# ziotom78/pytracer

Hardware: AMD Instinct MI355X
Metric: Mray/s (primary+shadow; rays handed to a world query) at 1280x720 per GPU, C2: 32 spheres + 1 plane, FlatRenderer (higher is better)
Workload: dtype f64; 1 GPU; C2 flat 1280x720, 32 spheres + 1 plane, S=0, every primary ray traced (dome shortcut off), fp32 RGB resident in HBM; width=1280, height=720, renderer=FlatRenderer

## Files before the change

pytracer_amd/csrc/pt_kernels.h:

```cpp
#pragma once
#include <hip/hip_runtime.h>
#include <stdint.h>

#include "../../include/ptrace.h"
#include "pt_layout.h"

#define PT_DEV static __device__ __forceinline__
#define PT_PI 3.141592653589793
#define PT_BLOCK 256
#ifndef PT_WAVES_SIMPLE
#define PT_WAVES_SIMPLE 4
#endif
#ifndef PT_WAVES_TILE
#define PT_WAVES_TILE 4
#endif
#ifndef PT_REGION
#define PT_REGION 8
#endif

typedef const __attribute__((address_space(4))) double *pt_kdouble;
typedef const __attribute__((address_space(4))) int32_t *pt_kint;
#define PT_KD(p) ((pt_kdouble)(const void *)(p))
#define PT_KI(p) ((pt_kint)(const void *)(p))

typedef const __attribute__((address_space(4))) PtKArgs *pt_kargs;
PT_DEV pt_kargs cold_args(const PtKArgs &a) {
  unsigned long long p = (unsigned long long)a.cold;
  asm volatile("" : "+s"(p));
  return (pt_kargs)p;
}

#ifndef PT_QUEUE_WORDS
#define PT_QUEUE_WORDS 512
#endif
#define PT_QUEUE_HEADS 256
#define PT_Q_CHOICE 200
#define PT_Q_HEAVY 201
#define PT_Q_BUDGET 202
#define PT_HANDOVER_HEADER 8
#ifndef PT_UNIT_SHARDS
#define PT_UNIT_SHARDS 8
#endif
static_assert(PT_QUEUE_HEADS + 32 * PT_UNIT_SHARDS <= PT_QUEUE_WORDS, "the shard heads must lie inside the queue block");
PT_DEV unsigned long long *pt_queue(const PtKArgs &a) { return cold_args(a)->queue + (size_t)a.qpar * PT_QUEUE_WORDS; }
PT_DEV unsigned long long *pt_queue_next(const PtKArgs &a) { return cold_args(a)->queue + (size_t)(a.qpar ^ 1) * PT_QUEUE_WORDS; }

struct V3 {
  double x, y, z;
};
struct Ray {
  V3 o, d;
  double tmin;
};
struct Hit {
  V3 wp, n;
  double u, v;
};

#include "pt_math.h"
#include "pt_query.h"
#include "pt_shade.h"
#include "pt_camera.h"
#include "pt_simple.h"
#include "pt_tile.h"
#include "pt_hits.h"
#include "pt_path.h"
#include "pt_tree.h"
#include "pt_probes.h"
```

pytracer_amd/csrc/pt_shade.h:

```cpp
template <bool INL = false, typename RP = const PtShapeRec *, typename AP = const PtShapeAux *>
PT_DEV void hit_details(RP rec, AP ax, const Ray &r, double t, Hit &h, bool need_uv) {
  double im[12];
#pragma unroll
  for (int k = 0; k < 12; ++k) im[k] = rec->invm[k];
  const V3 o = xf_point(im, r.o);
  const V3 d = xf_vec(im, r.d);
  const V3 hp = {o.x + t * d.x, o.y + t * d.y, o.z + t * d.z};
  double fm[12];
#pragma unroll
  for (int k = 0; k < 12; ++k) fm[k] = ax->m[k];
  h.wp = xf_point(fm, hp);
  V3 nn;
  h.u = 0.0;
  h.v = 0.0;
  if (rec->kind == PT_SHAPE_SPHERE) {
    const bool keep = dot3(hp, d) < 0.0;
    nn.x = keep ? hp.x : -hp.x;
    nn.y = keep ? hp.y : -hp.y;
    nn.z = keep ? hp.z : -hp.z;
    if (need_uv) {
      const double uu = pt_atan2(hp.y, hp.x) / (2.0 * PT_PI);
      h.u = (uu >= 0.0) ? uu : uu + 1.0;
      double z = hp.z;
      z = (z > 1.0) ? 1.0 : ((z < -1.0) ? -1.0 : z);
      h.v = pt_acos(z) / PT_PI;
    }
  } else {
    nn.x = 0.0;
    nn.y = 0.0;
    nn.z = (d.z < 0.0) ? 1.0 : -1.0;
    if (need_uv) {
      h.u = hp.x - floor(hp.x);
      h.v = hp.y - floor(hp.y);
    }
  }
  h.n = normalize3(xf_normal(im, nn));
}

template <typename CP>
PT_DEV V3 pigment_color(const PtKArgs &a, int kind, CP c1, CP c2, double steps, int tex, double u, double v) {
  if (kind == PT_PIGMENT_IMAGE) {
    pt_kargs ca = cold_args(a);
    const PtTex *tx = ca->tex + tex;
    const int w = tx->w, hh = tx->h;
    long long col = (long long)(u * (double)w);
    long long row = (long long)(v * (double)hh);
    if (col >= w) col = w - 1;
    if (row >= hh) row = hh - 1;
    const double *c = ca->tex_data + tx->offset + (row * w + col) * 3;
    V3 r = {c[0], c[1], c[2]};
    return r;
  }
  CP c = c1;
  if (kind == PT_PIGMENT_CHECKERED) {
    const double tu = floor(u * steps), tv = floor(v * steps);
    const bool odd_u = floor(tu * 0.5) * 2.0 != tu, odd_v = floor(tv * 0.5) * 2.0 != tv;
    c = (odd_u == odd_v) ? c1 : c2;
  }
  V3 r = {c[0], c[1], c[2]};
  return r;
}
template <typename AP>
PT_DEV V3 brdf_pigment(const PtKArgs &a, AP ax, double u, double v) {
  return pigment_color(a, ax->pig_kind, &ax->pig_c1[0], &ax->pig_c2[0], ax->pig_steps, ax->pig_tex, u, v);
}
template <typename AP>
PT_DEV V3 emitted_pigment(const PtKArgs &a, AP ax, double u, double v) {
  return pigment_color(a, ax->emi_kind, &ax->emi_c1[0], &ax->emi_c2[0], ax->emi_steps, ax->emi_tex, u, v);
}

template <bool INL = false>
PT_DEV Ray scatter_ray(int brdf_kind, Pcg &pcg, V3 incoming, V3 point, V3 n) {
  Ray r;
  r.o = point;
  if (brdf_kind == PT_BRDF_DIFFUSE) {
    const double sign = (n.z > 0.0) ? 1.0 : -1.0;
    const double aa = -1.0 / (sign + n.z);
    const double bb = n.x * n.y * aa;
    const V3 e1 = {1.0 + sign * n.x * n.x * aa, sign * bb, -sign * n.x};
    const V3 e2 = {bb, sign + n.y * n.y * aa, -n.y};
    const double cts = pcg_float(pcg);
    const double ct = sqrt(cts), st = sqrt(1.0 - cts);
    const double phi = 2.0 * PT_PI * pcg_float(pcg);
    double cp, sp;
    if (INL)
      sincos(phi, &sp, &cp);
    else
      pt_sincos(phi, &sp, &cp);
    r.d.x = ct * (cp * e1.x) + ct * (sp * e2.x) + st * n.x;
    r.d.y = ct * (cp * e1.y) + ct * (sp * e2.y) + st * n.y;
    r.d.z = ct * (cp * e1.z) + ct * (sp * e2.z) + st * n.z;
    r.tmin = 1.0e-3;
  } else {
    const V3 rd = normalize3(incoming);
    const V3 nn = normalize3(n);
    const double dp = dot3(nn, rd);
    r.d.x = rd.x - dp * (2.0 * nn.x);
    r.d.y = rd.y - dp * (2.0 * nn.y);
    r.d.z = rd.z - dp * (2.0 * nn.z);
    r.tmin = 1e-5;
  }
  return r;
}

PT_NOINLINE void scatter_ray_call(int brdf_kind, Pcg *pcg, const V3 *incoming, const V3 *point, const V3 *n, Ray *out) {
  *out = scatter_ray(brdf_kind, *pcg, *incoming, *point, *n);
}
```

pytracer_amd/csrc/pt_tile.h:

```cpp
struct TileCone {
  float ox, oy, oz;
  float ax, ay, az;
  float cos_t, sin_t;
  float oabs;
  bool all;
  float kx, ky, kz;
  float dmax2;
  float dmin;
  float rbeam;
  bool ortho;
};

struct ConeCam {
  float d0[3], dx[3], dy[3], apex[3];
  bool ortho;
};

PT_DEV ConeCam cone_cam(const PtKArgs &a) {
  ConeCam k;
  pt_kargs c = cold_args(a);
  for (int i = 0; i < 3; ++i) {
    k.d0[i] = c->cone_d0[i];
    k.dx[i] = c->cone_dx[i];
    k.dy[i] = c->cone_dy[i];
// ... 475 lines not shown
   bool strip_dome = block_dome, strip_settled = block_settled;
   if (use_strips && !block_dome) strip_dome = shared_cull(tx_first, tx_end, ty * 8, ty * 8 + 7, strip_cum, strip_settled);
   {
    const int tx = tx_first + wib;
    if (tx >= tx_end) continue;
    const int tile = ty * tiles_x + tx;
    PT_TSTAMP(7);
    const int col = tx * 8 + (lane & 7), lrow = ty * 8 + (lane >> 3);
    const bool active = col < W && lrow < rows_local;
    const int ccol = col < W ? col : W - 1, clrow = lrow < rows_local ? lrow : rows_local - 1;
    const long long pix = (long long)clrow * W + ccol;
    if (strip_dome) {
      if (strip_settled && active) {
        store_pixel(a, pix, KEEP ? dc_cum : strip_cum, out_f32);
        nrays += (unsigned long long)nsamp;
        nres += (unsigned long long)nsamp;
      }
      if (RENDERER == PT_RENDERER_PATHTRACER) {
        const unsigned long long todo = strip_settled ? 0ULL : __ballot(active);
        if (lane == 0) {
          rmask[tile] = todo;
          rkeys[tile] = (unsigned char)__popcll(todo);
            if (todo) note_flagged(pt_queue(a), __popcll(todo));
        }
      }
      continue;
    }
    const int pcol = ccol, grow = global_row(a, clrow);

    PT_TSTAMP(0);
    const int gr0 = global_row(a, ty * 8);
    const int gr1 = global_row(a, (ty * 8 + 7 < rows_local) ? ty * 8 + 7 : rows_local - 1);
    const float4 b_first = KEEP ? b_kept : a.bounds[(!HIER && lane < a.n_shapes) ? lane : 0];
    const TileCone tc = tile_cone(a, tx * 8, (tx * 8 + 8 < W) ? tx * 8 + 8 : W, gr0, gr1);
    PT_TSTAMP(1);
    int tpass = npass;
    const unsigned int *list = nullptr;
    int list_cnt = 0;
    int nsurv = 0, only = 0;
    bool dome_here = false;
    if (HIER) {
      const int cell = __builtin_amdgcn_readfirstlane((gr0 / PT_CELL) * a.cells_x + (tx * 8) / PT_CELL);
      const int cnt = PT_KI(a.cell_count)[cell];
      list_cnt = cnt;
      list = a.cell_list + (size_t)cell * a.cell_stride;
      tpass = (cnt + 63) >> 6;
      for (int p = 0; p < tpass; ++p) {
        const int idx = p * 64 + lane;
        bool keep = false;
        int slot = 0;
        float4 b = {0.0f, 0.0f, 0.0f, -1.0f};
        if (idx < cnt) {
          slot = (int)list[idx];
          b = a.bounds[slot];
        }
        const bool isplane = idx < cnt && slot >= a.n_spheres;
        if (idx < cnt && !isplane) keep = cone_keeps(tc, b);
        if (__any(isplane)) {
          const bool pk = plane_keeps(tc, b, isplane);
          if (isplane) keep = pk;
        }
        const unsigned long long m = __ballot(keep);
        if (lane == 0) pt_lds_masks[mbase + p] = m;
        nsurv += __popcll(m);
        if (m) only = (int)list[p * 64 + (__ffsll((long long)m) - 1)];
        if (RENDERER == PT_RENDERER_PATHTRACER && __ballot(keep && slot == dome_slot)) dome_here = true;
      }
    } else {
      for (int p = 0; p < npass; ++p) {
        const int slot = p * 64 + lane;
        bool keep = false;
        float4 b = {0.0f, 0.0f, 0.0f, -1.0f};
        if (slot < a.n_shapes) b = p == 0 ? b_first : a.bounds[slot];
        const bool isplane = slot >= a.n_spheres && slot < a.n_shapes;
        if (slot < a.n_spheres) keep = cone_keeps(tc, b);
        if (__any(isplane)) {
          const bool pk = plane_keeps(tc, b, isplane);
          if (isplane) keep = pk;
        }
        const unsigned long long m = __ballot(keep);
        if (lane == 0) pt_lds_masks[mbase + p] = m;
        nsurv += __popcll(m);
        if (m) only = p * 64 + (__ffsll((long long)m) - 1);
        if (RENDERER == PT_RENDERER_PATHTRACER && p == (dome_slot >> 6) && ((m >> (dome_slot & 63)) & 1ULL)) dome_here = true;
      }
    }
    __builtin_amdgcn_fence(__ATOMIC_RELEASE, "wavefront");
    __builtin_amdgcn_wave_barrier();
    __builtin_amdgcn_fence(__ATOMIC_ACQUIRE, "wavefront");
    PT_TSTAMP(2);

    if (dome_on && nsurv == 1 && only < a.n_spheres) {
      only = __builtin_amdgcn_readfirstlane(only);
      double hc_;
      float dmax2 = tc.dmax2, dmin = tc.dmin;
      if (ORTHO) {
        const float fro2 = (float)PT_KD(&a.recs[only])[13];
        pt_kdouble m = PT_KD(a.recs[only].invm);
        const float ox = (float)m[0] * tc.kx + (float)m[1] * tc.ky + (float)m[2] * tc.kz + (float)m[3];
        const float oy = (float)m[4] * tc.kx + (float)m[5] * tc.ky + (float)m[6] * tc.kz + (float)m[7];
        const float oz = (float)m[8] * tc.kx + (float)m[9] * tc.ky + (float)m[10] * tc.kz + (float)m[11];
        float o2 = ox * ox + oy * oy + oz * oz;
        o2 = fmaxf(o2, __shfl_xor(o2, 1, 64));
        o2 = fmaxf(o2, __shfl_xor(o2, 2, 64));
        const float slack = 1e-5f * (fro2 * (tc.oabs * tc.oabs * 3.0f + 1.0f) + 1.0f);
        hc_ = (o2 + slack < 0.45f) ? -0.55 : 0.0;
        pt_kargs cc_ = cold_args(a);
        const float d2 = cc_->cone_apex[0] * cc_->cone_apex[0] + cc_->cone_apex[1] * cc_->cone_apex[1] +
                         cc_->cone_apex[2] * cc_->cone_apex[2];
        dmax2 = d2 * (1.0f + 1e-5f);
        dmin = __fsqrt_rn(d2) * (1.0f - 1e-5f);
      } else {
        hc_ = 0.0;
      }
      V3 cum;
      bool settled;
      if (dome_value(only, hc_, dmax2, dmin, tc.all, cum, settled)) {
        if (settled && active) {
          store_pixel(a, pix, cum, out_f32);
          nrays += (unsigned long long)nsamp;
          nres += (unsigned long long)nsamp;
        }
        if (RENDERER == PT_RENDERER_PATHTRACER) {
          const unsigned long long todo = settled ? 0ULL : __ballot(active);
          if (lane == 0) {
            rmask[tile] = todo;
            rkeys[tile] = (unsigned char)__popcll(todo);
            if (todo) note_flagged(pt_queue(a), __popcll(todo));
          }
        }
        __builtin_amdgcn_wave_barrier();
        continue;
      }
    }

    if (RENDERER == PT_RENDERER_PATHTRACER && !ORTHO && dome_on && dome_here && nsurv > 1) {
      dome_prepare(dome_slot);
      if (dc_usable && dc_settled && dc_hc < -0.5 && dc_fro2 * tc.dmax2 < 1e6f && tc.dmin > 1e-6f && !tc.all) {
        const TileCone pc = pixel_cone(cone_cam(a), tc, pcol, grow);
        bool hitable = pc.all;
        for (int p = 0; p < tpass; ++p) {
          const unsigned long long mv = pt_lds_masks[mbase + p];
          const unsigned m_hi = (unsigned)__builtin_amdgcn_readfirstlane((int)(unsigned)(mv >> 32));
          const unsigned m_lo = (unsigned)__builtin_amdgcn_readfirstlane((int)(unsigned)mv);
          unsigned long long mask = ((unsigned long long)m_hi << 32) | (unsigned long long)m_lo;
          if (!mask) continue;
          const int myi = p * 64 + lane;
          int slot_q = myi;
          if (HIER) slot_q = myi < list_cnt ? (int)list[myi] : 0;
          const float4 bq = a.bounds[slot_q < a.n_shapes ? slot_q : 0];
          while (mask) {
            const int bit = __ffsll((long long)mask) - 1;
            mask &= mask - 1;
            const int slot = __builtin_amdgcn_readlane(slot_q, bit);
            if (slot == dome_slot) continue;
            if (slot >= a.n_spheres) {
              hitable = true;
            } else {
              const float4 b = {__int_as_float(__builtin_amdgcn_readlane(__float_as_int(bq.x), bit)),
                                __int_as_float(__builtin_amdgcn_readlane(__float_as_int(bq.y), bit)),
                                __int_as_float(__builtin_amdgcn_readlane(__float_as_int(bq.z), bit)),
                                __int_as_float(__builtin_amdgcn_readlane(__float_as_int(bq.w), bit))};
              hitable = hitable || cone_keeps(pc, b);
            }
          }
        }
        const V3 cum = dc_cum;
        if (active && !hitable) {
          store_pixel(a, pix, cum, out_f32);
          nrays += (unsigned long long)nsamp;
          nres += (unsigned long long)nsamp;
        }
        const unsigned long long todo = __ballot(active && hitable);
        if (lane == 0) {
          rmask[tile] = todo;
          rkeys[tile] = (unsigned char)__popcll(todo);
            if (todo) note_flagged(pt_queue(a), __popcll(todo));
        }
        __builtin_amdgcn_wave_barrier();
        continue;
      }
    }

    Pcg pcg;
    unsigned long long gpix = 0;
    if (S > 0) {
      pt_kargs c = cold_args(a);
      gpix = (unsigned long long)grow * c->W + pcol;
      pcg_seed_pixel(pcg, c->pcg_mode, c->s0, c->q0, gpix, nsamp);
    }
    V3 cum = {0.0, 0.0, 0.0};
    bool alive = active;
    int pix_rays = 0;
    for (int s = 0; s < nsamp; ++s) {
      if (RENDERER == PT_RENDERER_PATHTRACER && !__any(alive)) break;
      double up = 0.5, vp = 0.5;
      if (S > 0) {
        pt_kargs c = cold_args(a);
        if (c->pcg_mode == PT_PCG_SAMPLE) pcg_seed(pcg, c->s0, c->q0 + gpix * (unsigned)nsamp + (unsigned)s);
        const int sr = s / S, sc = s - sr * S;
        up = ((double)sc + pcg_float(pcg)) / (double)S;
        vp = ((double)sr + pcg_float(pcg)) / (double)S;
      }
      const Ray ray = primary_ray(a, pcol, grow, up, vp);
      PT_TSTAMP(3);
      double best_t;
      const int hit = world_query_tile<RENDERER == PT_RENDERER_ONOFF, HIER, !ORTHO>(a, ray, mbase, tpass, best_t, alive, list);
      PT_TSTAMP(4);
      if (alive) pix_rays++;
      V3 c;
      {
        pt_kargs ca = cold_args(a);
        c.x = ca->bg[0];
        c.y = ca->bg[1];
        c.z = ca->bg[2];
      }
      if (RENDERER == PT_RENDERER_ONOFF) {
        if (hit >= 0) {
          pt_kargs ca = cold_args(a);
          c.x = ca->onoff[0];
          c.y = ca->onoff[1];
          c.z = ca->onoff[2];
        }
      } else if (RENDERER == PT_RENDERER_POINTLIGHT) {
        unsigned long long shadow_rays = 0;
        c = pointlight_shade(a, ray, hit, best_t, alive, c, shadow_rays);
        pix_rays += (int)shadow_rays;
      } else if (RENDERER == PT_RENDERER_PATHTRACER) {
        if (hit >= 0) {
          pt_kargs ca = cold_args(a);
          const PtShapeAux *ax = ca->aux + hit;
          Hit h;
          h.u = 0.0;
          h.v = 0.0;
          if (ax->needs_uv) hit_details(a.recs + hit, ax, ray, best_t, h, true);
          const V3 hc = brdf_pigment(a, ax, h.u, h.v);
          const V3 em = emitted_pigment(a, ax, h.u, h.v);
          const double lum = max2(max2(hc.x, hc.y), hc.z);
          if (ca->rr <= 0 || lum > 0.0) alive = false;
          const double invN = 1.0 / (double)ca->N;
          c.x = em.x + 0.0 * invN;
          c.y = em.y + 0.0 * invN;
          c.z = em.z + 0.0 * invN;
        }
      } else {
        if (hit >= 0) {
          const PtShapeAux *ax = cold_args(a)->aux + hit;
          Hit h;
          h.u = 0.0;
          h.v = 0.0;
          if (ax->needs_uv) hit_details(a.recs + hit, ax, ray, best_t, h, true);
          const V3 p1 = brdf_pigment(a, ax, h.u, h.v);
          const V3 p2 = emitted_pigment(a, ax, h.u, h.v);
          c.x = p1.x + p2.x;
          c.y = p1.y + p2.y;
          c.z = p1.z + p2.z;
        }
      }
      if (S > 0) {
        cum.x = cum.x + c.x;
        cum.y = cum.y + c.y;
        cum.z = cum.z + c.z;
      } else {
        cum = c;
      }
      PT_TSTAMP(5);
    }
    if (S > 0) {
      const double k = 1.0 / (double)(S * S);
      cum.x = cum.x * k;
      cum.y = cum.y * k;
      cum.z = cum.z * k;
    }
    if (alive) {
      store_pixel(a, pix, cum, out_f32);
      nrays += (unsigned long long)pix_rays;
    }
    if (RENDERER == PT_RENDERER_PATHTRACER) {
      const unsigned long long todo = __ballot(active && !alive);
      if (lane == 0) {
        rmask[tile] = todo;
        rkeys[tile] = (unsigned char)__popcll(todo);
        if (todo) note_flagged(pt_queue(a), __popcll(todo));
      }
    }
    __builtin_amdgcn_wave_barrier();
    PT_TSTAMP(6);
   }
   }
  }
#ifdef PT_DEBUG_TIME
  if (RENDERER != PT_RENDERER_PATHTRACER && (threadIdx.x & 63) == 0 && (blockIdx.x & 63) == 0)
    for (int q = 0; q < 8; ++q) atomicAdd(pt_queue(a) + 1 + q, tsum[q]);
  pt_dbg_flush();
#endif
  add_ray_count(a, nrays, count_base, nres);
}

struct Hit4 {
  double best_t[4];
  int best[4];
};

template <bool ANYHIT>
PT_DEV void sphere_roots1(const PtKArgs &a, int slot, bool active, double tmin, double ox, double oy, double oz, double dx,
                          double dy, double dz, double aa, double cc, double &best_t, int &best) {
  const double tmax = INFINITY;
  PT_SPHERE_ROOTS(slot);
}

#ifndef PT_TILE4_WAVES
#define PT_TILE4_WAVES 4
#endif
template <int RENDERER, bool SLDS = false>
__global__ __launch_bounds__(PT_BLOCK) __attribute__((amdgpu_waves_per_eu(PT_TILE4_WAVES, 8))) void pt_tile4_kernel(const PtKArgs a) {
  constexpr int NPX = 4;
  constexpr int TH = 16;
  constexpr bool ANYHIT = RENDERER == PT_RENDERER_ONOFF;
#ifdef PT_DEBUG_TIME
  unsigned long long tsum[8] = {0, 0, 0, 0, 0, 0, 0, 0}, tprev = __builtin_amdgcn_s_memtime();
#define PT_T4(k) do { const unsigned long long tn = __builtin_amdgcn_s_memtime(); tsum[k] += tn - tprev; tprev = tn; } while (0)
#else
#define PT_T4(k) do { } while (0)
#endif
  int W, rows_local, npass;
  bool dome_on, out_f32;
  {
    pt_kargs c = cold_args(a);
    out_f32 = c->out_f32 != 0;
    W = c->W;
    rows_local = c->rows_local;
    npass = c->npass;
    dome_on = c->dome_shortcut != 0;
  }
  const int lane = threadIdx.x & 63, wib = threadIdx.x >> 6;
  const int tx = blockIdx.x * 2 + (wib & 1), ty = blockIdx.y * 2 + (wib >> 1);
  unsigned long long nrays = 0, nres = 0;
  const bool valid = tx * 16 < W && ty * TH < rows_local;
  if (SLDS) {
    const unsigned long long *src = (const unsigned long long *)a.recs;
    for (int k = threadIdx.x; k < a.n_shapes * 16; k += PT_BLOCK) pt_lds_masks[k] = src[k];
    src = (const unsigned long long *)a.aux;
    for (int k = threadIdx.x; k < a.n_shapes * 32; k += PT_BLOCK) pt_lds_masks[a.n_shapes * 16 + k] = src[k];
    __syncthreads();
  }
  if (valid) {
    const int lr0 = ty * TH, lr1 = (lr0 + TH - 1 < rows_local) ? lr0 + TH - 1 : rows_local - 1;
    const int gr0 = global_row(a, lr0);
    const float4 b_first = a.bounds[lane < a.n_shapes ? lane : 0];
    PT_T4(0);
    const TileCone tc = tile_cone(a, tx * 16, (tx * 16 + 16 < W) ? tx * 16 + 16 : W, gr0, gr0 + (lr1 - lr0));
    PT_T4(1);
    unsigned long long masks[4] = {0ULL, 0ULL, 0ULL, 0ULL};
    int nsurv = 0, only = 0;
#pragma unroll
    for (int p = 0; p < 4; ++p) {
      if (p < npass) {
        const int slot = p * 64 + lane;
        bool keep = false;
        float4 b = {0.0f, 0.0f, 0.0f, -1.0f};
        if (slot < a.n_shapes) b = p == 0 ? b_first : a.bounds[slot];
        const bool isplane = slot >= a.n_spheres && slot < a.n_shapes;
        if (slot < a.n_spheres) keep = cone_keeps(tc, b);
        if (__any(isplane)) {
          const bool pk = plane_keeps(tc, b, isplane);
          if (isplane) keep = pk;
        }
        const unsigned long long m = __ballot(keep);
        masks[p] = m;
        nsurv += __popcll(m);
        if (m) only = p * 64 + (__ffsll((long long)m) - 1);
      }
    }
    PT_T4(2);
    const int colA = tx * 16 + (lane & 7), colB = colA + 8;
    const int lrowA = lr0 + (lane >> 3), lrowB = lrowA + 8;
    const bool okcA = colA < W, okcB = colB < W, okrA = lrowA < rows_local, okrB = lrowB < rows_local;
    const bool act[4] = {okcA && okrA, okcB && okrA, okcA && okrB, okcB && okrB};
    const int ccA = okcA ? colA : W - 1, ccB = okcB ? colB : W - 1;
    const int crA = okrA ? lrowA : rows_local - 1, crB = okrB ? lrowB : rows_local - 1;
    const long long pix[4] = {(long long)crA * W + ccA, (long long)crA * W + ccB, (long long)crB * W + ccA, (long long)crB * W + ccB};
    bool done = false;
    if (dome_on && nsurv == 1 && only < a.n_spheres) {
      only = __builtin_amdgcn_readfirstlane(only);
      pt_kargs ca = cold_args(a);
      const PtShapeAux *ax = ca->aux + only;
      const float fro2 = (float)PT_KD(&a.recs[only])[13];
      const double hc = (only < a.n_diag) ? PT_KD(&a.hoist_diag[only])[6] : PT_KD(&a.hoist[only])[3];
      if (ax->needs_uv == 0 && hc < -0.5 && fro2 * tc.dmax2 < 1e6f && tc.dmin > 1e-6f && !tc.all) {
        V3 c;
        if (RENDERER == PT_RENDERER_ONOFF) {
          c.x = ca->onoff[0];
          c.y = ca->onoff[1];
          c.z = ca->onoff[2];
        } else {
          const V3 p1 = brdf_pigment(a, ax, 0.0, 0.0), p2 = emitted_pigment(a, ax, 0.0, 0.0);
          c.x = p1.x + p2.x;
          c.y = p1.y + p2.y;
          c.z = p1.z + p2.z;
        }
#pragma unroll
        for (int k = 0; k < NPX; ++k)
          if (act[k]) {
            store_pixel(a, pix[k], c, out_f32);
            nrays += 1ULL;
            nres += 1ULL;
          }
        done = true;
      }
    }
    PT_T4(3);
    if (!done) {
      V3 org, dir[4];
      double bgx, bgy, bgz;
      {
        pt_kargs c = cold_args(a);
        const double dist = c->cam_dist, aspect = c->cam_aspect;
        const double Wd = (double)c->W, Hd = (double)c->H;
        const int growA = gr0 + (crA - lr0), growB = gr0 + (crB - lr0);
        const double uA = ((double)ccA + 0.5) / Wd, uB = ((double)ccB + 0.5) / Wd;
        const double vA = 1.0 - ((double)growA + 0.5) / Hd, vB = 1.0 - ((double)growB + 0.5) / Hd;
        const double dyA = (1.0 - 2.0 * uA) * aspect, dyB = (1.0 - 2.0 * uB) * aspect;
        const double dzA = 2.0 * vA - 1.0, dzB = 2.0 * vB - 1.0;
        const double m0 = c->cam_m[0], m1 = c->cam_m[1], m2 = c->cam_m[2], m3 = c->cam_m[3];
        const double m4 = c->cam_m[4], m5 = c->cam_m[5], m6 = c->cam_m[6], m7 = c->cam_m[7];
        const double m8 = c->cam_m[8], m9 = c->cam_m[9], m10 = c->cam_m[10], m11 = c->cam_m[11];
        const double xA = dist * m0 + dyA * m1, xB = dist * m0 + dyB * m1;
        const double yA = dist * m4 + dyA * m5, yB = dist * m4 + dyB * m5;
        const double zA = dist * m8 + dyA * m9, zB = dist * m8 + dyB * m9;
        dir[0] = {xA + dzA * m2, yA + dzA * m6, zA + dzA * m10};
        dir[1] = {xB + dzA * m2, yB + dzA * m6, zB + dzA * m10};
        dir[2] = {xA + dzB * m2, yA + dzB * m6, zA + dzB * m10};
        dir[3] = {xB + dzB * m2, yB + dzB * m6, zB + dzB * m10};
        const double ox_ = -dist, oy_ = 0.0, oz_ = 0.0;
        org.x = ox_ * m0 + oy_ * m1 + oz_ * m2 + m3;
        org.y = ox_ * m4 + oy_ * m5 + oz_ * m6 + m7;
        org.z = ox_ * m8 + oy_ * m9 + oz_ * m10 + m11;
        bgx = c->bg[0];
        bgy = c->bg[1];
        bgz = c->bg[2];
      }
      PT_T4(4);
      const double tmin = 1.0e-5;
      Hit4 h4;
      bool fast = true;
#pragma unroll
      for (int k = 0; k < NPX; ++k) {
        h4.best_t[k] = INFINITY;
        h4.best[k] = -1;
        Ray rk;
        rk.o = org;
        rk.d = dir[k];
        rk.tmin = tmin;
        fast = fast && wave_guard<true>(rk, act[k]).fast;
      }
      const int nd = a.n_diag, ns = a.n_spheres;
      bool all_hit = false;
#pragma unroll
      for (int p = 0; p < 4; ++p) {
        unsigned long long mask = masks[p];
        while (mask && !all_hit) {
          const int slot = p * 64 + (__ffsll((long long)mask) - 1);
          mask &= mask - 1;
          if (slot < ns) {
            if (slot < nd && fast) {
              pt_kdouble h = PT_KD(&a.hoist_diag[slot]);
              const double s0 = h[0], s1 = h[1], s2 = h[2], ox = h[3], oy = h[4], oz = h[5], cc = h[6];
#pragma unroll
              for (int k = 0; k < NPX; ++k) {
                const double dx = dir[k].x * s0, dy = dir[k].y * s1, dz = dir[k].z * s2;
                const double aa = dx * dx + dy * dy + dz * dz;
                sphere_roots1<ANYHIT>(a, slot, act[k], tmin, ox, oy, oz, dx, dy, dz, aa, cc, h4.best_t[k], h4.best[k]);
              }
            } else {
              pt_kdouble m = PT_KD(a.recs[slot].invm);
              pt_kdouble h = PT_KD(&a.hoist[slot]);
              const double ox = h[0], oy = h[1], oz = h[2], cc = h[3];
#pragma unroll
              for (int k = 0; k < NPX; ++k) {
                const double dx = dir[k].x * m[0] + dir[k].y * m[1] + dir[k].z * m[2];
                const double dy = dir[k].x * m[4] + dir[k].y * m[5] + dir[k].z * m[6];
                const double dz = dir[k].x * m[8] + dir[k].y * m[9] + dir[k].z * m[10];
                const double aa = dx * dx + dy * dy + dz * dz;
                sphere_roots1<ANYHIT>(a, slot, act[k], tmin, ox, oy, oz, dx, dy, dz, aa, cc, h4.best_t[k], h4.best[k]);
              }
            }
          } else {
            pt_kdouble m = PT_KD(a.recs[slot].invm);
            const double oz = PT_KD(&a.hoist[slot])[2];
            const double tmax = INFINITY;
#pragma unroll
            for (int k = 0; k < NPX; ++k) {
              const double dz = dir[k].x * m[8] + dir[k].y * m[9] + dir[k].z * m[10];
              const bool active = act[k];
              double &best_t = h4.best_t[k];
              int &best = h4.best[k];
              PT_PLANE_HIT(slot);
            }
          }
          if (ANYHIT) {
            const bool open = (act[0] && h4.best[0] < 0) || (act[1] && h4.best[1] < 0) || (act[2] && h4.best[2] < 0) ||
                              (act[3] && h4.best[3] < 0);
            all_hit = __ballot(open) == 0ULL;
          }
        }
      }
      PT_T4(5);
#pragma unroll
      for (int k = 0; k < NPX; ++k) {
        V3 c = {bgx, bgy, bgz};
        const int hit = h4.best[k];
        if (RENDERER == PT_RENDERER_ONOFF) {
          if (hit >= 0) {
            pt_kargs ca = cold_args(a);
            c.x = ca->onoff[0];
            c.y = ca->onoff[1];
            c.z = ca->onoff[2];
          }
        } else if (hit >= 0) {
          Hit h;
          h.u = 0.0;
          h.v = 0.0;
          Ray rk;
          rk.o = org;
          rk.d = dir[k];
          rk.tmin = tmin;
          V3 p1, p2;
          if constexpr (SLDS) {
            const pt_lds_rec rec = (pt_lds_rec)(const void *)pt_lds_f64 + hit;
            const pt_lds_aux ax = (pt_lds_aux)(const void *)(pt_lds_f64 + a.n_shapes * 16) + hit;
            if (ax->needs_uv) {
              hit_details(rec, ax, rk, h4.best_t[k], h, true);
              p1 = brdf_pigment(a, ax, h.u, h.v);
              p2 = emitted_pigment(a, ax, h.u, h.v);
              c.x = p1.x + p2.x;
              c.y = p1.y + p2.y;
              c.z = p1.z + p2.z;
            } else {
              c.x = ax->pig_c2[0];
              c.y = ax->pig_c2[1];
              c.z = ax->pig_c2[2];
            }
          } else {
            const PtShapeAux *ax = cold_args(a)->aux + hit;
            if (ax->needs_uv) {
              hit_details(a.recs + hit, ax, rk, h4.best_t[k], h, true);
              p1 = brdf_pigment(a, ax, h.u, h.v);
              p2 = emitted_pigment(a, ax, h.u, h.v);
              c.x = p1.x + p2.x;
              c.y = p1.y + p2.y;
              c.z = p1.z + p2.z;
            } else {
              c.x = ax->pig_c2[0];
              c.y = ax->pig_c2[1];
              c.z = ax->pig_c2[2];
            }
          }
        }
        PT_T4(6);
        if (act[k]) {
          store_pixel(a, pix[k], c, out_f32);
          nrays += 1ULL;
        }
        PT_T4(7);
      }
    }
  }
#ifdef PT_DEBUG_TIME
#ifdef PT_DEBUG_HEAVY
  {
    unsigned long long tot_ = 0;
    for (int q = 0; q < 8; ++q) tot_ += tsum[q];
    if ((threadIdx.x & 63) == 0 && ((blockIdx.y * gridDim.x + blockIdx.x) & 3) == 0 && tot_ > PT_DEBUG_HEAVY)
      for (int q = 0; q < 8; ++q) atomicAdd(pt_queue(a) + 1 + q, tsum[q]);
  }
#else
  if ((threadIdx.x & 63) == 0 && ((blockIdx.y * gridDim.x + blockIdx.x) & 15) == 0)
    for (int q = 0; q < 8; ++q) atomicAdd(pt_queue(a) + 1 + q, tsum[q]);
#endif
  if ((threadIdx.x & 63) == 0) {
    const int wv = (blockIdx.y * gridDim.x + blockIdx.x) * 4 + (int)(threadIdx.x >> 6);
    if (wv < PT_UNITLOG_LEN) {
      unsigned long long tot_ = 0;
      for (int q = 0; q < 8; ++q) tot_ += tsum[q];
      pt_unitlog[wv * 8] = tot_;
      pt_unitlog[wv * 8 + 1] = tsum[0] + tsum[1] + tsum[2] + tsum[3];
      pt_unitlog[wv * 8 + 2] = __builtin_amdgcn_s_memtime();
    }
  }
  if ((threadIdx.x & 63) == 0 && ((blockIdx.y * gridDim.x + blockIdx.x) & 15) == 0) {
    unsigned long long tot = 0;
    for (int q = 0; q < 8; ++q) tot += tsum[q];
    atomicMax(pt_queue(a) + 12, tot);
    if (tot > 16384ULL) atomicAdd(pt_queue(a) + 13, 1ULL);
    if (tot > 24576ULL) atomicAdd(pt_queue(a) + 14, 1ULL);
    if (tot > 32768ULL) atomicAdd(pt_queue(a) + 15, 1ULL);
  }
#endif
  add_ray_count(a, nrays, 0, nres, blockIdx.y * gridDim.x + blockIdx.x);
}
```

Baseline: 65890 Mray/s.

## Shade tile4 hits per shape with wave-uniform loop over winning shapes

Replaces per-pixel divergent shading in the tile4 kernel with a loop that picks one surviving shape per iteration via ballot/readlane and shades all matching pixels with wave-uniform (scalar) shape data, using precomputed hoisted origins and a batched pigment helper. It is used when few shapes survive (nsurv <= 2) and falls back to the old per-pixel path otherwise. It also raises the waves-per-EU hint from 4 to 5 and drops the nres counter in favour of a settled flag. The intent is to cut divergence and per-lane scattered loads during shading, at the cost of extra loop iterations, more code size and possible register-pressure changes.

Result: faster. 69740 Mray/s (median of 6 runs) (+5.8%).

```diff
diff --git a/pytracer_amd/csrc/pt_kernels.h b/pytracer_amd/csrc/pt_kernels.h
--- a/pytracer_amd/csrc/pt_kernels.h
+++ b/pytracer_amd/csrc/pt_kernels.h
@@ -13,6 +13,9 @@
 #endif
 #ifndef PT_WAVES_TILE
 #define PT_WAVES_TILE 4
+#endif
+#ifndef PT_T4_MUTANT
+#define PT_T4_MUTANT 0
 #endif
 #ifndef PT_REGION
 #define PT_REGION 8
diff --git a/pytracer_amd/csrc/pt_shade.h b/pytracer_amd/csrc/pt_shade.h
--- a/pytracer_amd/csrc/pt_shade.h
+++ b/pytracer_amd/csrc/pt_shade.h
@@ -69,6 +69,48 @@
   return pigment_color(a, ax->emi_kind, &ax->emi_c1[0], &ax->emi_c2[0], ax->emi_steps, ax->emi_tex, u, v);
 }
 
+template <int N>
+PT_DEV void pigment_color_n(const PtKArgs &a, int kind, pt_kdouble c1, pt_kdouble c2, double steps, int tex, const double (&u)[N],
+                            const double (&v)[N], const bool (&on)[N], V3 (&out)[N]) {
+  if (kind == PT_PIGMENT_IMAGE) {
+    pt_kargs ca = cold_args(a);
+    const PtTex *tx = ca->tex + tex;
+    const int w = tx->w, hh = tx->h;
+    const double *base = ca->tex_data + tx->offset;
+#pragma unroll
+    for (int k = 0; k < N; ++k) {
+      out[k] = {0.0, 0.0, 0.0};
+      if (on[k]) {
+        long long col = (long long)(u[k] * (double)w);
+        long long row = (long long)(v[k] * (double)hh);
+        if (col >= w) col = w - 1;
+        if (row >= hh) row = hh - 1;
+        const double *c = base + (row * w + col) * 3;
+        out[k] = {c[0], c[1], c[2]};
+      }
+    }
+    return;
+  }
+  const double c1x = c1[0], c1y = c1[1], c1z = c1[2];
+  if (kind == PT_PIGMENT_CHECKERED) {
+    const double c2x = c2[0], c2y = c2[1], c2z = c2[2];
+#pragma unroll
+    for (int k = 0; k < N; ++k) {
+      const double tu = floor(u[k] * steps), tv = floor(v[k] * steps);
+      const bool odd_u = floor(tu * 0.5) * 2.0 != tu, odd_v = floor(tv * 0.5) * 2.0 != tv;
+#if PT_T4_MUTANT == 2
+      const bool first = odd_u != odd_v;
+#else
+      const bool first = odd_u == odd_v;
+#endif
+      out[k] = {first ? c1x : c2x, first ? c1y : c2y, first ? c1z : c2z};
+    }
+    return;
+  }
+#pragma unroll
+  for (int k = 0; k < N; ++k) out[k] = {c1x, c1y, c1z};
+}
+
 template <bool INL = false>
 PT_DEV Ray scatter_ray(int brdf_kind, Pcg &pcg, V3 incoming, V3 point, V3 n) {
   Ray r;
diff --git a/pytracer_amd/csrc/pt_tile.h b/pytracer_amd/csrc/pt_tile.h
--- a/pytracer_amd/csrc/pt_tile.h
+++ b/pytracer_amd/csrc/pt_tile.h
@@ -801,6 +801,15 @@
   int best[4];
 };
 
+PT_DEV V3 t4_origin(double dist, pt_kdouble m) {
+  const double ox_ = -dist, oy_ = 0.0, oz_ = 0.0;
+  V3 org;
+  org.x = ox_ * m[0] + oy_ * m[1] + oz_ * m[2] + m[3];
+  org.y = ox_ * m[4] + oy_ * m[5] + oz_ * m[6] + m[7];
+  org.z = ox_ * m[8] + oy_ * m[9] + oz_ * m[10] + m[11];
+  return org;
+}
+
 template <bool ANYHIT>
 PT_DEV void sphere_roots1(const PtKArgs &a, int slot, bool active, double tmin, double ox, double oy, double oz, double dx,
                           double dy, double dz, double aa, double cc, double &best_t, int &best) {
@@ -808,8 +817,11 @@
   PT_SPHERE_ROOTS(slot);
 }
 
+#ifndef PT_T4_WINNERS
+#define PT_T4_WINNERS 2
+#endif
 #ifndef PT_TILE4_WAVES
-#define PT_TILE4_WAVES 4
+#define PT_TILE4_WAVES 5
 #endif
 template <int RENDERER, bool SLDS = false>
 __global__ __launch_bounds__(PT_BLOCK) __attribute__((amdgpu_waves_per_eu(PT_TILE4_WAVES, 8))) void pt_tile4_kernel(const PtKArgs a) {
@@ -818,7 +830,7 @@
   constexpr bool ANYHIT = RENDERER == PT_RENDERER_ONOFF;
 #ifdef PT_DEBUG_TIME
   unsigned long long tsum[8] = {0, 0, 0, 0, 0, 0, 0, 0}, tprev = __builtin_amdgcn_s_memtime();
-#define PT_T4(k) do { const unsigned long long tn = __builtin_amdgcn_s_memtime(); tsum[k] += tn - tprev; tprev = tn; } while (0)
+#define PT_T4(k) do { __builtin_amdgcn_sched_barrier(0); const unsigned long long tn = __builtin_amdgcn_s_memtime(); tsum[k] += tn - tprev; tprev = tn; __builtin_amdgcn_sched_barrier(0); } while (0)
 #else
 #define PT_T4(k) do { } while (0)
 #endif
@@ -834,7 +846,8 @@
   }
   const int lane = threadIdx.x & 63, wib = threadIdx.x >> 6;
   const int tx = blockIdx.x * 2 + (wib & 1), ty = blockIdx.y * 2 + (wib >> 1);
-  unsigned long long nrays = 0, nres = 0;
+  unsigned long long nrays = 0;
+  bool settled = false;
   const bool valid = tx * 16 < W && ty * TH < rows_local;
   if (SLDS) {
     const unsigned long long *src = (const unsigned long long *)a.recs;
@@ -903,9 +916,9 @@
           if (act[k]) {
             store_pixel(a, pix[k], c, out_f32);
             nrays += 1ULL;
-            nres += 1ULL;
           }
         done = true;
+        settled = true;
       }
     }
     PT_T4(3);
@@ -921,9 +934,9 @@
         const double vA = 1.0 - ((double)growA + 0.5) / Hd, vB = 1.0 - ((double)growB + 0.5) / Hd;
         const double dyA = (1.0 - 2.0 * uA) * aspect, dyB = (1.0 - 2.0 * uB) * aspect;
         const double dzA = 2.0 * vA - 1.0, dzB = 2.0 * vB - 1.0;
-        const double m0 = c->cam_m[0], m1 = c->cam_m[1], m2 = c->cam_m[2], m3 = c->cam_m[3];
-        const double m4 = c->cam_m[4], m5 = c->cam_m[5], m6 = c->cam_m[6], m7 = c->cam_m[7];
-        const double m8 = c->cam_m[8], m9 = c->cam_m[9], m10 = c->cam_m[10], m11 = c->cam_m[11];
+        const double m0 = c->cam_m[0], m1 = c->cam_m[1], m2 = c->cam_m[2];
+        const double m4 = c->cam_m[4], m5 = c->cam_m[5], m6 = c->cam_m[6];
+        const double m8 = c->cam_m[8], m9 = c->cam_m[9], m10 = c->cam_m[10];
         const double xA = dist * m0 + dyA * m1, xB = dist * m0 + dyB * m1;
         const double yA = dist * m4 + dyA * m5, yB = dist * m4 + dyB * m5;
         const double zA = dist * m8 + dyA * m9, zB = dist * m8 + dyB * m9;
@@ -931,10 +944,7 @@
         dir[1] = {xB + dzA * m2, yB + dzA * m6, zB + dzA * m10};
         dir[2] = {xA + dzB * m2, yA + dzB * m6, zA + dzB * m10};
         dir[3] = {xB + dzB * m2, yB + dzB * m6, zB + dzB * m10};
-        const double ox_ = -dist, oy_ = 0.0, oz_ = 0.0;
-        org.x = ox_ * m0 + oy_ * m1 + oz_ * m2 + m3;
-        org.y = ox_ * m4 + oy_ * m5 + oz_ * m6 + m7;
-        org.z = ox_ * m8 + oy_ * m9 + oz_ * m10 + m11;
+        org = t4_origin(dist, PT_KD(c->cam_m));
         bgx = c->bg[0];
         bgy = c->bg[1];
         bgz = c->bg[2];
@@ -1005,62 +1015,178 @@
         }
       }
       PT_T4(5);
-#pragma unroll
-      for (int k = 0; k < NPX; ++k) {
-        V3 c = {bgx, bgy, bgz};
-        const int hit = h4.best[k];
-        if (RENDERER == PT_RENDERER_ONOFF) {
-          if (hit >= 0) {
+      if constexpr (RENDERER == PT_RENDERER_ONOFF) {
+#pragma unroll
+        for (int k = 0; k < NPX; ++k) {
+          V3 c = {bgx, bgy, bgz};
+          if (h4.best[k] >= 0) {
             pt_kargs ca = cold_args(a);
             c.x = ca->onoff[0];
             c.y = ca->onoff[1];
             c.z = ca->onoff[2];
           }
-        } else if (hit >= 0) {
-          Hit h;
-          h.u = 0.0;
-          h.v = 0.0;
-          Ray rk;
-          rk.o = org;
-          rk.d = dir[k];
-          rk.tmin = tmin;
-          V3 p1, p2;
-          if constexpr (SLDS) {
-            const pt_lds_rec rec = (pt_lds_rec)(const void *)pt_lds_f64 + hit;
-            const pt_lds_aux ax = (pt_lds_aux)(const void *)(pt_lds_f64 + a.n_shapes * 16) + hit;
-            if (ax->needs_uv) {
-              hit_details(rec, ax, rk, h4.best_t[k], h, true);
-              p1 = brdf_pigment(a, ax, h.u, h.v);
-              p2 = emitted_pigment(a, ax, h.u, h.v);
-              c.x = p1.x + p2.x;
-              c.y = p1.y + p2.y;
-              c.z = p1.z + p2.z;
+          PT_T4(6);
+          if (act[k]) {
+            store_pixel(a, pix[k], c, out_f32);
+            nrays += 1ULL;
+          }
+          PT_T4(7);
+        }
+      } else {
+        auto put = [&](int k, const V3 &c) {
+          int l = lane;
+          asm volatile("" : "+v"(l));
+          const int col = tx * 16 + (l & 7) + ((k & 1) ? 8 : 0), row = lr0 + (l >> 3) + ((k & 2) ? 8 : 0);
+          const int cc = col < W ? col : W - 1, cr = row < rows_local ? row : rows_local - 1;
+          store_pixel(a, (long long)cr * W + cc, c, out_f32);
+        };
+        int open[4];
+#pragma unroll
+        for (int k = 0; k < NPX; ++k) open[k] = h4.best[k];
+        if (nsurv <= PT_T4_WINNERS) {
+#pragma unroll 1
+          for (;;) {
+            const int c01 = open[0] > open[1] ? open[0] : open[1], c23 = open[2] > open[3] ? open[2] : open[3];
+            const int cand = c01 > c23 ? c01 : c23;
+            const unsigned long long left = __ballot(cand >= 0);
+            if (left == 0ULL) break;
+            const int s = __builtin_amdgcn_readlane(cand, __ffsll((long long)left) - 1);
+            const PtShapeAux *axs = a.aux + s;
+            bool on[4];
+#pragma unroll
+            for (int k = 0; k < NPX; ++k) on[k] = open[k] == s;
+            if (*PT_KI(&axs->needs_uv) == 0) {
+              pt_kdouble c2 = PT_KD(axs->pig_c2);
+              const V3 c = {c2[0], c2[1], c2[2]};
+              PT_T4(6);
+#pragma unroll
+              for (int k = 0; k < NPX; ++k)
+                if (on[k]) put(k, c);
+              PT_T4(7);
             } else {
-              c.x = ax->pig_c2[0];
-              c.y = ax->pig_c2[1];
-              c.z = ax->pig_c2[2];
+              pt_kdouble im = PT_KD(a.recs[s].invm);
+              pt_kdouble ho = PT_KD(&a.hoist[s]);
+              const V3 o = {ho[0], ho[1], ho[2]};
+              const bool sphere = *PT_KI(&a.recs[s].kind) == PT_SHAPE_SPHERE;
+              const int pig_kind = *PT_KI(&axs->pig_kind), emi_kind = *PT_KI(&axs->emi_kind);
+#pragma unroll
+              for (int h = 0; h < NPX; h += 2) {
+                double u[2], v[2];
+                const bool on2[2] = {on[h], on[h + 1]};
+                if (sphere) {
+#pragma unroll
+                  for (int j = 0; j < 2; ++j) {
+                    u[j] = 0.0;
+                    v[j] = 0.0;
+                    if (on2[j]) {
+                      const V3 d = xf_vec(im, dir[h + j]);
+                      const double t = h4.best_t[h + j];
+                      const V3 hp = {o.x + t * d.x, o.y + t * d.y, o.z + t * d.z};
+                      const double uu = pt_atan2(hp.y, hp.x) / (2.0 * PT_PI);
+                      u[j] = (uu >= 0.0) ? uu : uu + 1.0;
+                      double z = hp.z;
+                      z = (z > 1.0) ? 1.0 : ((z < -1.0) ? -1.0 : z);
+                      v[j] = pt_acos(z) / PT_PI;
+                    }
+                  }
+                } else {
+#pragma unroll
+                  for (int j = 0; j < 2; ++j) {
+                    const V3 d = xf_vec(im, dir[h + j]);
+                    const double t = h4.best_t[h + j];
+                    const double hx = o.x + t * d.x, hy = o.y + t * d.y;
+                    u[j] = hx - floor(hx);
+                    v[j] = hy - floor(hy);
+                  }
+                }
+                V3 ck[2], p2[2];
+                pigment_color_n<2>(a, pig_kind, PT_KD(axs->pig_c1), PT_KD(axs->pig_c2), *PT_KD(&axs->pig_steps), *PT_KI(&axs->pig_tex), u, v, on2, ck);
+                pigment_color_n<2>(a, emi_kind, PT_KD(axs->emi_c1), PT_KD(axs->emi_c2), *PT_KD(&axs->emi_steps), *PT_KI(&axs->emi_tex), u, v, on2, p2);
+#if PT_T4_MUTANT != 3
+#pragma unroll
+                for (int j = 0; j < 2; ++j) ck[j] = {ck[j].x + p2[j].x, ck[j].y + p2[j].y, ck[j].z + p2[j].z};
+#endif
+                PT_T4(6);
+#pragma unroll
+                for (int j = 0; j < 2; ++j)
+                  if (on2[j]) put(h + j, ck[j]);
+                PT_T4(7);
+                __builtin_amdgcn_sched_barrier(0);
+              }
             }
-          } else {
-            const PtShapeAux *ax = cold_args(a)->aux + hit;
-            if (ax->needs_uv) {
-              hit_details(a.recs + hit, ax, rk, h4.best_t[k], h, true);
-              p1 = brdf_pigment(a, ax, h.u, h.v);
-              p2 = emitted_pigment(a, ax, h.u, h.v);
-              c.x = p1.x + p2.x;
-              c.y = p1.y + p2.y;
-              c.z = p1.z + p2.z;
-            } else {
-              c.x = ax->pig_c2[0];
-              c.y = ax->pig_c2[1];
-              c.z = ax->pig_c2[2];
+#pragma unroll
+            for (int k = 0; k < NPX; ++k) open[k] = on[k] ? -2 : open[k];
+          }
+        } else {
+#if PT_T4_MUTANT != 1
+#pragma unroll
+          for (int k = 0; k < NPX; ++k) {
+            const int hit = open[k];
+            V3 c = {0.0, 0.0, 0.0};
+            if (hit >= 0) {
+              Hit h;
+              h.u = 0.0;
+              h.v = 0.0;
+              Ray rk;
+              pt_kargs ca = cold_args(a);
+              rk.o = t4_origin(ca->cam_dist, PT_KD(ca->cam_m));
+              rk.d = dir[k];
+              rk.tmin = tmin;
+              V3 p1, p2;
+              if constexpr (SLDS) {
+                const pt_lds_rec rec = (pt_lds_rec)(const void *)pt_lds_f64 + hit;
+                const pt_lds_aux ax = (pt_lds_aux)(const void *)(pt_lds_f64 + a.n_shapes * 16) + hit;
+                if (ax->needs_uv) {
+                  hit_details(rec, ax, rk, h4.best_t[k], h, true);
+                  p1 = brdf_pigment(a, ax, h.u, h.v);
+                  p2 = emitted_pigment(a, ax, h.u, h.v);
+                  c.x = p1.x + p2.x;
+                  c.y = p1.y + p2.y;
+                  c.z = p1.z + p2.z;
+                } else {
+                  c.x = ax->pig_c2[0];
+                  c.y = ax->pig_c2[1];
+                  c.z = ax->pig_c2[2];
+                }
+              } else {
+                const PtShapeAux *ax = cold_args(a)->aux + hit;
+                if (ax->needs_uv) {
+                  hit_details(a.recs + hit, ax, rk, h4.best_t[k], h, true);
+                  p1 = brdf_pigment(a, ax, h.u, h.v);
+                  p2 = emitted_pigment(a, ax, h.u, h.v);
+                  c.x = p1.x + p2.x;
+                  c.y = p1.y + p2.y;
+                  c.z = p1.z + p2.z;
+                } else {
+                  c.x = ax->pig_c2[0];
+                  c.y = ax->pig_c2[1];
+                  c.z = ax->pig_c2[2];
+                }
+              }
+#ifndef PT_DEBUG_TIME
+              put(k, c);
+#endif
             }
+#ifdef PT_DEBUG_TIME
+            PT_T4(6);
+            if (hit >= 0) put(k, c);
+            PT_T4(7);
+#endif
           }
+#endif
         }
         PT_T4(6);
-        if (act[k]) {
-          store_pixel(a, pix[k], c, out_f32);
-          nrays += 1ULL;
-        }
+        const V3 bg = {bgx, bgy, bgz};
+#pragma unroll
+        for (int k = 0; k < NPX; ++k)
+          if (act[k]) {
+#if PT_T4_MUTANT == 1
+            if (open[k] != -2) put(k, bg);
+#else
+            if (open[k] == -1) put(k, bg);
+#endif
+            nrays += 1ULL;
+          }
         PT_T4(7);
       }
     }
@@ -1096,5 +1222,5 @@
     if (tot > 32768ULL) atomicAdd(pt_queue(a) + 15, 1ULL);
   }
 #endif
-  add_ray_count(a, nrays, 0, nres, blockIdx.y * gridDim.x + blockIdx.x);
+  add_ray_count(a, nrays, 0, settled ? nrays : 0ULL, blockIdx.y * gridDim.x + blockIdx.x);
 }
```
